# locuslab/mpc.pytorch

Measured on AMD Instinct MI355X. Metric: LQR problem-steps/sec (batch*T/s), n_state=12 n_ctrl=4 T=50, higher is better.
Workload: dtype f32

## Files before the change

include/mpc_lqr.h:

```cpp
#ifndef MPC_LQR_H
#define MPC_LQR_H

#include <stdint.h>

#ifdef __cplusplus
extern "C" {
#endif

#define MPC_LQR_ABI_VERSION 9

enum { MPC_F32 = 0, MPC_F64 = 1 };
enum { MPC_BOUND_NONE = 0, MPC_BOUND_SCALAR = 1, MPC_BOUND_TENSOR = 2 };
enum {
    MPC_OK = 0,
    MPC_E_DIMS = -1,
    MPC_E_NULL = -2,
    MPC_E_DTYPE = -3,
    MPC_E_LAUNCH = -4,
    MPC_E_ARG = -5,
    MPC_E_UNSUPPORTED = -6
};
enum {
    MPC_ST_PNQP_UNCONVERGED = 1,
    MPC_ST_NONFINITE = 2,
// ... 65 lines not shown
    void *k;
} mpc_lqr_outputs;

int mpc_lqr_abi_version(void);
const char *mpc_lqr_build_info(void);
const char *mpc_lqr_last_error(void);

int64_t mpc_lqr_workspace_bytes(const mpc_lqr_problem *p);

int mpc_lqr_step(const mpc_lqr_problem *p, const mpc_lqr_options *o, const mpc_lqr_outputs *out,
                 void *workspace, int64_t workspace_bytes, int impl, void *stream);

int mpc_lqr_step_route(const mpc_lqr_problem *p, const mpc_lqr_options *o, const mpc_lqr_outputs *out,
                       const void *workspace, int64_t workspace_bytes, int impl, int *ring);

int mpc_lqr_qp_record(const mpc_lqr_problem *p, const mpc_lqr_options *o, int impl, int64_t *offset_bytes, int64_t *st, int64_t *sb);

int mpc_lqr_impl_supported(const mpc_lqr_problem *p, const mpc_lqr_options *o, int impl);

int mpc_lqr_sweep(const mpc_lqr_problem *p, const mpc_lqr_options *o, const mpc_lqr_outputs *out,
                  void *stream);

int mpc_lqr_rollout(const mpc_lqr_problem *p, const mpc_lqr_options *o, const mpc_lqr_outputs *out,
                    const void *old_costs_in, void *stream);

int mpc_lqr_kkt_grads(const mpc_lqr_problem *p,
                      const void *dx, const void *du, const void *dl_dx, const void *dl_du,
                      void *dC, void *dc, void *dF, void *df, void *dx_init, void *stream);

enum { MPC_KKT_GRADS_DPP16 = 1, MPC_KKT_GRADS_WAVE = 2, MPC_KKT_GRADS_GENERIC = 3 };
// ... 106 lines not shown
```

mpc.pytorch_amd/csrc/capi.hip:

```cpp
#include <algorithm>
#include <cmath>
#include <cstdio>
#include <cstdlib>
#include <cstring>
#include <string>

#include "lqr_common.h"

namespace mpclqr {
static thread_local std::string g_last_error;
void set_last_error(const char *msg) { g_last_error = msg ? msg : ""; }

static int fail(int code, const char *msg)
{
    set_last_error(msg);
    return code;
}

struct DeviceFacts {
    int ring_force;
    int simds;
    int ring40_force;
    bool sticky;
};
static const DeviceFacts &device_facts()
{
    static DeviceFacts f = [] {
        DeviceFacts d;
        d.ring_force = 0;
        d.ring40_force = 0;
        d.simds = 1024;
        hipDeviceProp_t prop;
        int dev = 0;
        if (hipGetDevice(&dev) == hipSuccess && hipGetDeviceProperties(&prop, dev) == hipSuccess && prop.multiProcessorCount > 0)
            d.simds = prop.multiProcessorCount * 4;
        const char *force = getenv("MPC_DPP16_RING");
        if (force && (force[0] == '2' || force[0] == '4')) d.ring_force = force[0] - '0';
        const char *force40 = getenv("MPC_MFMA40_RING");
        if (force40 && (force40[0] == '2' || force40[0] == '3')) d.ring40_force = force40[0] - '0';
        d.sticky = getenv("MPC_DPP16_RING_DYNAMIC") == nullptr;
        return d;
    }();
    return f;
}
static int dpp16_ring_force()
{
    const DeviceFacts &f = device_facts();
    if (f.sticky) return f.ring_force;
    const char *force = getenv("MPC_DPP16_RING");
    return (force && (force[0] == '2' || force[0] == '4')) ? force[0] - '0' : 0;
}

static int mfma40_ring(const StepParams<float> &sp)
{
    const DeviceFacts &f = device_facts();
    int force = f.ring40_force;
    if (!f.sticky) {
        const char *e = getenv("MPC_MFMA40_RING");
        force = (e && (e[0] == '2' || e[0] == '3')) ? e[0] - '0' : 0;
    }
    if (force) return force;
    if (sp.bound_mode != MPC_BOUND_NONE) return sp.B > f.simds ? 2 : 3;
    return (sp.B > f.simds && sp.B <= f.simds + f.simds / 2) ? 2 : 3;
}

// ... 299 lines not shown
    sp.gate = sp.status;
    sp.Kk = nullptr;
    if (!sp.K || !sp.k) {
        const WsLayout w = ws_layout<real>(MPC_IMPL_GENERIC, sp.T, sp.B, sp.ns, sp.nc);
        sp.K = (real *)((char *)workspace + w.K);
        sp.k = (real *)((char *)workspace + w.k);
    }
    return launch_step_generic<real>(sp, sp.sweep_only ? 1 : 3, st);
}

static int launch_routed(const StepRoute &r, const StepParams<float> &q, hipStream_t st)
{
    switch (r.kernel) {
    case MPC_IMPL_GENERIC: return launch_step_generic<float>(q, r.phase, st);
    case MPC_IMPL_MFMA16: return launch_step_mfma16(q, st);
    case MPC_IMPL_DPP16: return r.ring == 2 ? launch_step_dpp16_ring2(q, st) : launch_step_dpp16(q, st);
    case MPC_IMPL_TINY: return launch_step_tiny<float>(q, st);
    case MPC_IMPL_MFMA40: return r.ring == 2 ? launch_step_mfma40_ring2(q, st) : launch_step_mfma40(q, st);
    case MPC_IMPL_WAVE1: return launch_step_wave1(q, st);
    case MPC_IMPL_MFMA40_PAD: return r.pad16 ? launch_step_mfma40_pad16(q, st) : launch_step_mfma40_pad4(q, st);
    case MPC_IMPL_DPP16_PAD: return launch_step_dpp16_pad(q, st);
    case MPC_IMPL_MFMA40_NARROW: return r.pad16 ? launch_step_mfma40_narrow16(q, st) : launch_step_mfma40_narrow4(q, st);
    }
    return MPC_E_ARG;
}
static int launch_routed(const StepRoute &r, const StepParams<double> &q, hipStream_t st)
{
    switch (r.kernel) {
    case MPC_IMPL_GENERIC: return launch_step_generic<double>(q, r.phase, st);
    case MPC_IMPL_MFMA16: return launch_step_mfma16(q, st);
    case MPC_IMPL_TINY: return launch_step_tiny<double>(q, st);
// ... 238 lines not shown
    if (!p) return 0;
    return status_scratch_offset(p) + (int64_t)p->B * 4 + 256;
}

int mpc_lqr_step(const mpc_lqr_problem *p, const mpc_lqr_options *o, const mpc_lqr_outputs *out,
                 void *workspace, int64_t workspace_bytes, int impl, void *stream)
{
    const int rc = check_step(p, o, out);
    if (rc) return rc;
    if (p->B == 0) return MPC_OK;
    hipStream_t st = (hipStream_t)stream;
    return p->dtype == MPC_F32 ? step_impl<float>(p, o, out, workspace, workspace_bytes, impl, 3, nullptr, st)
                               : step_impl<double>(p, o, out, workspace, workspace_bytes, impl, 3, nullptr, st);
}

int mpc_lqr_step_route(const mpc_lqr_problem *p, const mpc_lqr_options *o, const mpc_lqr_outputs *out, const void *workspace,
                       int64_t workspace_bytes, int impl, int *ring)
{
    const int rc = check_step(p, o, out);
    if (rc) return rc;
    if (ring) *ring = 0;
    if (p->B == 0) return 0;
    return p->dtype == MPC_F32 ? route_query<float>(p, o, out, workspace, workspace_bytes, impl, ring)
                               : route_query<double>(p, o, out, workspace, workspace_bytes, impl, ring);
}

int mpc_lqr_impl_supported(const mpc_lqr_problem *p, const mpc_lqr_options *o, int impl)
{
    if (!p || check_problem(p, false, false) != MPC_OK || check_options(p, o) != MPC_OK) return 0;
    if (impl < MPC_IMPL_GENERIC || impl > MPC_IMPL_MFMA40_NARROW) return 0;
// ... 453 lines not shown
```

mpc.pytorch_amd/csrc/lqr_common.h:

```cpp
#pragma once
#include <hip/hip_runtime.h>
#include <stdint.h>
#include "../../include/mpc_lqr.h"
#include "lqr_params.h"

namespace mpclqr {

void set_last_error(const char *msg);

enum { MPC_IMPL_AUTO = 0, MPC_IMPL_GENERIC = 1, MPC_IMPL_MFMA16 = 2, MPC_IMPL_DPP16 = 3, MPC_IMPL_TINY = 4, MPC_IMPL_MFMA40 = 5,
       MPC_IMPL_WAVE1 = 6, MPC_IMPL_MFMA40_PAD = 7, MPC_IMPL_DPP16_PAD = 8,
       MPC_IMPL_MFMA40_NARROW = 9 };

struct StepRoute {
    int code; const char *msg;
    int kernel;
    int phase;
    int ring;
    bool pad16;
    bool needs_resolve;
    int64_t K_off, k_off;
    int64_t Kk_off, status_off;
    int64_t qp_off, qp_st, qp_sb;
};
// ... 33 lines not shown
                                                real *bd, void *flags, void *host_flags, int host_tag, const int *status,
                                                hipStream_t st);
template <typename real> int launch_du_norm_reference(int T, int B, int nc, const real *u, const real *new_u, real *out, hipStream_t st);
template <typename real> int launch_env_linearize(const EnvDesc<real> &env, long N, const real *x, const real *u,
                                                  real *F, real *f, hipStream_t st);
int64_t env_param_grad_workspace_bytes(int64_t N);
template <typename real> int launch_env_param_grad(const EnvDesc<real> &env, long N, const real *x, const real *u,
                                                   const real *gF, const real *gf, real *gparams, double *ws, hipStream_t st);
size_t generic_lds_bytes(int ns, int nc, size_t elem);
template <typename real> int launch_slew_augment(const mpc_lqr_problem *p, double gamma, real *aC, real *ac, real *aF, real *af, hipStream_t st);

bool dpp16_supported(const StepParams<float> &p);
int launch_step_dpp16(const StepParams<float> &p, hipStream_t st);
int launch_step_dpp16_ring2(const StepParams<float> &p, hipStream_t st);
bool dpp16_pad_supported(const StepParams<float> &p);
int launch_step_dpp16_pad(const StepParams<float> &p, hipStream_t st);
bool kkt_dpp16_supported(const StepParams<float> &p, const float *dx, const float *du, const float *dl_dx,
                         const float *dC, const float *dF);
int launch_kkt_dpp16(const StepParams<float> &p, const float *dx, const float *du, const float *dl_dx, float *dC,
                     float *dc, float *dF, float *df, float *dx_init, hipStream_t st);

bool kkt_fused_dpp16_supported(const StepParams<float> &p, const float *dl_dx, const float *dl_du, const float *dC,
                               const float *dF, const float *ws);
int64_t kkt_fused_dpp16_workspace_bytes(int T, int B);
bool kkt_fused_dpp16_pad_supported(const StepParams<float> &p, const float *ws);
int launch_kkt_fused_dpp16_pad(const StepParams<float> &p, const float *dl_dx, const float *dl_du, float *dC, float *dc, float *dF,
                               float *df, float *dx_init, float *dx_out, float *du_out, float *ws, float decay, int max_ls,
                               hipStream_t st);
int launch_kkt_fused_dpp16(const StepParams<float> &p, const float *dl_dx, const float *dl_du, float *dC, float *dc, float *dF,
                           float *df, float *dx_init, float *dx_out, float *du_out, float *ws, float decay, int max_ls,
// ... 76 lines not shown
```

mpc.pytorch_amd/csrc/lqr_dpp16.hip:

```cpp
#include <string>
#include "lqr_common.h"

#define MPC_DEV __device__ __forceinline__
#define DPPM " row_mask:0xf bank_mask:0xf\n"

namespace mpclqr {
namespace wv {
typedef float f32x4 __attribute__((ext_vector_type(4)));
MPC_DEV int lane() { return (int)threadIdx.x; }
MPC_DEV int problem() { return (int)blockIdx.x; }
MPC_DEV unsigned long long clock() { return (unsigned long long)clock64(); }
MPC_DEV float rcp(float x) { return __builtin_amdgcn_rcpf(x); }
MPC_DEV void pin(float &x) { asm volatile("" : "+v"(x)); }
MPC_DEV bool uniform(bool c) { return c; }
MPC_DEV int uniform(int v) { return v; }
MPC_DEV bool any(bool c) { return __ballot(c) != 0ull; }
MPC_DEV unsigned long long ballot(bool c) { return __ballot(c); }
MPC_DEV float readlane(float x, int l) { return __int_as_float(__builtin_amdgcn_readlane(__float_as_int(x), __builtin_amdgcn_readfirstlane(l))); }
MPC_DEV double readlane_f64(double x, int l)
{
    const unsigned long long b = __double_as_longlong(x);
    const int ll = __builtin_amdgcn_readfirstlane(l);
    const unsigned lo = (unsigned)__builtin_amdgcn_readlane((int)(unsigned)b, ll), hi = (unsigned)__builtin_amdgcn_readlane((int)(unsigned)(b >> 32), ll);
    return __longlong_as_double(((unsigned long long)hi << 32) | lo);
// ... 272 lines not shown
}
MPC_DEV double row_sum_f64(double x)
{
    x += mov_dpp_f64<0xB1>(x);
    x += mov_dpp_f64<0x4E>(x);
    x += mov_dpp_f64<0x141>(x);
    x += mov_dpp_f64<0x140>(x);
    return x;
}

#ifndef MPC_DPP16_NSTAGE
#define MPC_DPP16_NSTAGE 4
#endif
#ifdef MPC_KF_LDS_BYTES
#define MPC_DPP16_LDS (MPC_KF_LDS_BYTES)
#else
#define MPC_DPP16_LDS (MPC_DPP16_NSTAGE * 9216)
#endif
#ifndef MPC_KKT16_NSTAGE
#define MPC_KKT16_NSTAGE 4
#endif
#if !defined(MPC_DPP16_WITH_KKT) && !defined(MPC_DPP16_NO_KKT) && MPC_DPP16_NSTAGE == 4
#define MPC_DPP16_WITH_KKT 1
#endif
__shared__ __attribute__((aligned(16))) char g_stage16[MPC_DPP16_LDS];
typedef __attribute__((address_space(3))) void lds_void_t;
typedef __attribute__((address_space(1))) const void glb_void_t;
#ifndef MPC_DPP16_C_AUX
#define MPC_DPP16_C_AUX 2
#endif
// ... 243 lines not shown
    return true;
}

#endif

#ifndef MPC_DPP16_PAD_KKT
#ifdef MPC_DPP16_PAD
#define MPC_DPP16_LAUNCH launch_step_dpp16_pad
bool dpp16_pad_supported(const StepParams<float> &p)
{
    return p.ns >= 1 && p.ns <= 12 && p.nc >= 1 && p.nc <= 4 && p.T >= 1 && p.max_ls >= 1 && p.max_ls <= 16 && !p.env.kind;
}
#define MPC_DPP16_TAKES(p) dpp16_pad_supported(p)
#elif MPC_DPP16_NSTAGE == 4
#define MPC_DPP16_LAUNCH launch_step_dpp16
#else
#define MPC_DPP16_LAUNCH launch_step_dpp16_ring2
bool dpp16_supported(const StepParams<float> &p);
#endif
int MPC_DPP16_LAUNCH(const StepParams<float> &p, hipStream_t st)
{
#ifndef MPC_DPP16_TAKES
#define MPC_DPP16_TAKES(p) dpp16_supported(p)
#endif
    if (!MPC_DPP16_TAKES(p)) { set_last_error(dpp16::PADK ? "dpp16 (padded): needs fp32, n_state <= 12, n_ctrl <= 4, max_linesearch_iter <= 16" : "dpp16: needs n_state = 12, n_ctrl = 4, fp32, 16-byte aligned blocks"); return MPC_E_DIMS; }
    if (!p.Kk || (uintptr_t)p.Kk % 16 != 0) { set_last_error("dpp16: gain workspace missing or misaligned"); return MPC_E_NULL; }
    if (!p.sweep_only && (!p.new_x || !p.new_u)) { set_last_error("dpp16: new_x / new_u is NULL"); return MPC_E_NULL; }
    static_assert(MPC_DPP16_LDS == dpp16::LDS_TOTAL, "LDS layout out of sync");
    const dim3 grid((p.B + 3) / 4), block(64);
    if (p.bound_mode != MPC_BOUND_NONE) hipLaunchKernelGGL((lqr_step_dpp16_kernel<2>), grid, block, 0, st, p);
    else if (p.zero_mask) hipLaunchKernelGGL((lqr_step_dpp16_kernel<1>), grid, block, 0, st, p);
    else if (p.T <= dpp16::RG_STEPS) hipLaunchKernelGGL((lqr_step_dpp16_kernel<0>), grid, block, 0, st, p);
    else hipLaunchKernelGGL((lqr_step_dpp16_kernel<3>), grid, block, 0, st, p);
    hipError_t e = hipGetLastError();
    if (e != hipSuccess) {
        set_last_error((std::string("lqr_step_dpp16_kernel: ") + hipGetErrorString(e)).c_str());
        return MPC_E_LAUNCH;
    }
    return MPC_OK;
}
#endif

}
```

mpc.pytorch_amd/csrc/lqr_dpp16_body.h:

```cpp
#pragma once
#include <math.h>
#include "lqr_params.h"
#include "lqr_small_math.h"

#ifndef MPC_STAT
#define MPC_STAT(i)
#endif

#ifndef MPC_DEVM
#define MPC_DEVM MPC_DEV
#endif

#ifndef MPC_DPP16_NSTAGE
#define MPC_DPP16_NSTAGE 4
#endif
#ifndef MPC_DPP16_QP_WARM
#define MPC_DPP16_QP_WARM 0
#endif

#ifdef MPC_DPP16_PAD
#define MPC_DPP16_PADK 1
#else
#define MPC_DPP16_PADK 0
#endif
// ... 194 lines not shown
    fr_out[2] = wv::bcast<8>(mv) != 0.f; fr_out[3] = wv::bcast<12>(mv) != 0.f;
    converged = conv != 0.f;
    return (int)it_ret;
}

enum {
    SC = 0, SF = 4096, SR = 7168, SG = 8192, STAGE_BYTES = 9216, NSTAGE = MPC_DPP16_NSTAGE, AHEAD = NSTAGE - 1,
    R_c = 0, R_tau = 64, R_f = 128, R_qs = 176, R_lo = 192, R_hi = 208,
    LDS_TOTAL = NSTAGE * STAGE_BYTES,
#if defined(MPC_PAD_PROBE_DUP) && MPC_DPP16_PADK
    DMA_SWEEP = 48
#else
    DMA_SWEEP = MPC_DPP16_PADK ? 32 : 8
#endif
};
#if defined(MPC_PAD_PROBE_DUP) && MPC_DPP16_PADK
#define MPC_PAD_NF 12
#define MPC_PAD_NC 32
#else
#define MPC_PAD_NF 12
#define MPC_PAD_NC 16
#endif
template <int MODE, bool DIRECT> struct RollDma { enum { N = (MPC_DPP16_PADK ? MPC_PAD_NF + 4 : 3 + 1) + (rgm(MODE) ? 0 : 1) + (DIRECT ? (MPC_DPP16_PADK ? MPC_PAD_NC : 4) : (con(MODE) ? 1 : 0)) }; };
template <int MODE, bool DIRECT> struct RollRing {
    enum {
        BYTES = DIRECT ? (int)STAGE_BYTES : (con(MODE) ? 6144 : (rgm(MODE) ? 4096 : 5120)),
#ifdef MPC_DPP16_RSLOTS
        SLOTS = DIRECT ? (int)NSTAGE : (MPC_DPP16_RSLOTS),
#else
        SLOTS = DIRECT ? (int)NSTAGE : (int)LDS_TOTAL / (con(MODE) ? 6144 : (rgm(MODE) ? 4096 : 5120)),
// ... 15 lines not shown
    wv::lds_sync();
    for (unsigned off = 16u * (unsigned)lane; off + 16 <= bytes; off += 1024) wv::lds_store_f32x4(off, f32x4{0.f, 0.f, 0.f, 0.f});
    wv::lds_sync();
}

MPC_DEV int quarter_swizzle(int row) { return (row >> 1) & 3; }
MPC_DEV int src_granule_rows(int g) { return (g & ~3) | ((g & 3) ^ quarter_swizzle(g >> 2)); }
MPC_DEV int src_granule_cols(int g, int problem_slot) { return g ^ ((problem_slot & 1) << 2); }
MPC_DEV int src_granule_C(int g, int problem_slot)
{
#ifdef MPC_DPP16_NO_CPERM
    problem_slot = 0;
#endif
    const int R = (g >> 2) ^ (problem_slot & 3);
    return 4 * R + ((g & 3) ^ quarter_swizzle(R));
}

struct Lane {
    int lane, p, j;
    int pb;
    int b0;
    bool live;
    bool isu;
    bool ovalid;
    float padd[4];
    int a;
    int aCq[4];
    int aCcol;
    int aFe, aFo;
    int aFq[4];
// ... 205 lines not shown
        else if (K == 1) { MPC_PAD_C(8); MPC_PAD_C(9); MPC_PAD_C(10); MPC_PAD_C(11); MPC_PAD_C(12); MPC_PAD_C(13); MPC_PAD_C(14); MPC_PAD_C(15); }
        else if (K == 2) { MPC_PAD_F(0); MPC_PAD_F(1); MPC_PAD_F(2); MPC_PAD_F(3); MPC_PAD_F(4); MPC_PAD_F(5); MPC_PAD_F(6); MPC_PAD_F(7); }
        else { MPC_PAD_F(8); MPC_PAD_F(9); MPC_PAD_F(10); MPC_PAD_F(11); MPC_PAD_R(0); MPC_PAD_R(1); MPC_PAD_R(2); MPC_PAD_R(3); }
    } else {
        if (K == 0) { MPC_PAD_F(0); MPC_PAD_F(1); MPC_PAD_F(2); MPC_PAD_F(3); MPC_PAD_F(4); MPC_PAD_F(5); }
        else if (K == 1) { MPC_PAD_F(6); MPC_PAD_F(7); MPC_PAD_F(8); MPC_PAD_F(9); MPC_PAD_F(10); MPC_PAD_F(11); }
        else if (K == 2) { MPC_PAD_R(0); MPC_PAD_R(1); MPC_PAD_R(2); MPC_PAD_R(3); }
    }
#undef MPC_PAD_C
#undef MPC_PAD_F
#undef MPC_PAD_R
}
#endif

template <int MODE, bool ROLL, bool DIRECT>
MPC_DEV void stage_issue(const Dma &d, unsigned mid)
{
#ifdef MPC_DPP16_PAD
    pad_part<MODE, ROLL, DIRECT, 0>(d, mid); pad_part<MODE, ROLL, DIRECT, 1>(d, mid);
    pad_part<MODE, ROLL, DIRECT, 2>(d, mid); pad_part<MODE, ROLL, DIRECT, 3>(d, mid);
    if (ROLL && !rgm(MODE)) {
        if (DIRECT) wv::dma16_at<0>(d.g_ptr - 1024, mid + (SG - SF));
        else wv::dma16_at<-1024>(d.g_ptr, mid);
    }
    if (ROLL && !DIRECT && con(MODE)) wv::dma16_at<-2048>(d.g2_ptr, mid);
    return;
#endif
    if (!ROLL || DIRECT) {
        wv::dma16_at<-4096, wv::DMA_C>(d.c_ptr[0], mid);
        wv::dma16_at<-3072, wv::DMA_C>(d.c_ptr[1], mid);
        wv::dma16_at<-2048, wv::DMA_C>(d.c_ptr[2], mid);
        wv::dma16_at<-1024, wv::DMA_C>(d.c_ptr[3], mid);
    }
    wv::dma16_at<0, ROLL ? wv::DMA_LAST : wv::DMA_PLAIN>(d.f_ptr[0], mid);
    wv::dma16_at<1024, ROLL ? wv::DMA_LAST : wv::DMA_PLAIN>(d.f_ptr[1], mid);
    wv::dma16_at<2048, ROLL ? wv::DMA_LAST : wv::DMA_PLAIN>(d.f_ptr[2], mid);
    wv::dma16_at<3072>(d.r_ptr, mid);
    if (ROLL && !rgm(MODE)) {
        if (DIRECT) {
            wv::dma16_at<0>(d.g_ptr - 1024, mid + (SG - SF));
        } else {
            wv::dma16_at<-1024>(d.g_ptr, mid);
            if (con(MODE)) wv::dma16_at<-2048>(d.g2_ptr, mid);
        }
    }
}

template <int MODE, bool ROLL, bool DIRECT>
MPC_DEV void stage_move(Dma &d, bool move_f)
{
#ifdef MPC_DPP16_PAD
// ... 27 lines not shown
        if (con(MODE) && !DIRECT) d.g2_ptr += d.g2_step;
    }
}

template <int K, int ND> MPC_DEV void tail_wait(int rem)
{
    if (K == 0 || rem >= K) wv::dma_wait<K * ND>();
    else tail_wait<(K > 0 ? K - 1 : 0), ND>(rem);
}

template <int MODE, bool ROLL, bool DIRECT> struct Feed {
    Dma &d;
    unsigned mid;
    bool on;
    bool move_f;
    template <int K> MPC_DEVM void part()
    {
        if (!on) return;
#ifdef MPC_DPP16_PAD
        pad_part<MODE, ROLL, DIRECT, K>(d, mid);
        if (ROLL && !DIRECT) {
            if (K == 2) {
                if (!rgm(MODE)) wv::dma16_at<-1024>(d.g_ptr, mid);
                if (con(MODE)) wv::dma16_at<-2048>(d.g2_ptr, mid);
            } else if (K == 3) {
                stage_move<MODE, ROLL, DIRECT>(d, move_f);
            }
        } else if (K == 3) {
            if (ROLL && !rgm(MODE)) wv::dma16_at<0>(d.g_ptr - 1024, mid + (SG - SF));
            stage_move<MODE, ROLL, DIRECT>(d, move_f);
        }
        return;
#endif
        enum { NC = (!ROLL || DIRECT) ? 4 : 0 };
        if (ROLL && !DIRECT) {
            if (K == 0) {
                wv::dma16_at<0, wv::DMA_LAST>(d.f_ptr[0], mid);
                wv::dma16_at<1024, wv::DMA_LAST>(d.f_ptr[1], mid);
            } else if (K == 1) {
                wv::dma16_at<2048, wv::DMA_LAST>(d.f_ptr[2], mid);
                wv::dma16_at<3072>(d.r_ptr, mid);
            } else if (K == 2) {
                if (!rgm(MODE)) wv::dma16_at<-1024>(d.g_ptr, mid);
                if (con(MODE)) wv::dma16_at<-2048>(d.g2_ptr, mid);
            } else {
                stage_move<MODE, ROLL, DIRECT>(d, move_f);
            }
        } else {
            if (K == 0) {
                wv::dma16_at<-4096, wv::DMA_C>(d.c_ptr[0], mid);
                wv::dma16_at<-3072, wv::DMA_C>(d.c_ptr[1], mid);
            } else if (K == 1) {
                wv::dma16_at<-2048, wv::DMA_C>(d.c_ptr[2], mid);
                wv::dma16_at<-1024, wv::DMA_C>(d.c_ptr[3], mid);
            } else if (K == 2) {
// ... 380 lines not shown
    const f32x4 r = s.rec;
    const float k0 = wv::bcast<12>(r[0]), k1 = wv::bcast<12>(r[1]), k2 = wv::bcast<12>(r[2]), k3 = wv::bcast<12>(r[3]);
    const int a = L.a;
    s.kk = a == 0 ? k0 : (a == 1 ? k1 : (a == 2 ? k2 : k3));
    const float q00 = wv::bcast<13>(r[2]);
    const float q01 = wv::bcast<13>(r[0]), q11 = wv::bcast<13>(r[1]);
    const float q02 = wv::bcast<14>(r[0]), q12 = wv::bcast<14>(r[1]), q22 = wv::bcast<14>(r[2]);
    const float q03 = wv::bcast<15>(r[0]), q13 = wv::bcast<15>(r[1]), q23 = wv::bcast<15>(r[2]), q33 = wv::bcast<15>(r[3]);
    s.Sr[0] = a == 0 ? q00 : (a == 1 ? q01 : (a == 2 ? q02 : q03));
    s.Sr[1] = a == 0 ? q01 : (a == 1 ? q11 : (a == 2 ? q12 : q13));
    s.Sr[2] = a == 0 ? q02 : (a == 1 ? q12 : (a == 2 ? q22 : q23));
    s.Sr[3] = a == 0 ? q03 : (a == 1 ? q13 : (a == 2 ? q23 : q33));
}

template <int MODE, bool DIRECT>
MPC_DEV void ro_read(RoStage &s, const P &p, const Lane &L, int t, int slot, unsigned zm)
{
    const unsigned base = stage_mid<MODE, true, DIRECT>(slot) - SF;
    const unsigned mrec = base + RollRing<MODE, DIRECT>::MADJ;
    const unsigned gain = base + RollRing<MODE, DIRECT>::GADJ;
    s.cj = 0.f;
    if (DIRECT) {
#pragma unroll
        for (int q = 0; q < 4; ++q) {
            const f32x4 v = wv::lds_f32x4(base + L.aCq[q]);
            s.Cr[4 * q] = v[0]; s.Cr[4 * q + 1] = v[1]; s.Cr[4 * q + 2] = v[2]; s.Cr[4 * q + 3] = v[3];
        }
        s.cj = wv::lds_f32(base + L.aRec + R_c);
    } else {
#pragma unroll
        for (int b = 0; b < 4; ++b) s.Sr[b] = rgm(MODE) ? 0.f : wv::lds_f32(gain + L.aS[b]);
        if (con(MODE)) {
            const f32x4 mc = wv::lds_f32x4(L.j == 12 ? mrec + L.aMcol : gain + L.aGcol);
            const unsigned fm = wv::f32_bits(wv::lds_f32(gain + L.aFm));
#pragma unroll
            for (int a = 0; a < 4; ++a) s.Mc[a] = (L.j == 12 || !((fm >> a) & 1u)) ? mc[a] : 0.f;
        }
    }
#pragma unroll
    for (int q = 0; q < 4; ++q) {
        const f32x4 v = wv::lds_f32x4(base + L.aFq[q]);
        s.Fr[4 * q] = v[0]; s.Fr[4 * q + 1] = v[1]; s.Fr[4 * q + 2] = v[2]; s.Fr[4 * q + 3] = v[3];
    }
    s.fj = p.f ? wv::lds_f32(base + L.aRecF) : 0.f;
    if (!rgm(MODE)) {
#pragma unroll
        for (int jj = 0; jj < 12; ++jj) s.Kr[jj] = wv::lds_f32(gain + L.aKrow + 16 * jj);
        if (con(MODE)) {
            const unsigned fm = wv::f32_bits(wv::lds_f32(gain + L.aFm));
            const bool free_a = ((fm >> L.a) & 1u) != 0u;
#pragma unroll
            for (int jj = 0; jj < 12; ++jj) s.Kr[jj] = free_a ? s.Kr[jj] : 0.f;
        }
        s.kk = wv::lds_f32(gain + L.aKrow + 192);
    } else {
        s.kk = 0.f;
// ... 9 lines not shown
            s.lo = pad ? 0.f : p.lo_s;
            s.hi = pad ? 0.f : p.hi_s;
        }
    }
    s.zm = ((zm >> (8 * L.a)) & 0xffu) != 0u;
}

struct RoState {
    float xs;
    float cost, du2;
    float alpha;
    float pred;
    float viol;
    float *out;
    bool price_on;
    float xs1, cost1, du21;
    float *out1;
};

template <int MODE>
MPC_DEV float control_law(const P &p, const Lane &L, const RoStage &s, float xs, float alpha, float &e, float &dx)
{
    dx = L.isu ? 0.f : xs - s.tb;
    float un;
    if (rgm(MODE)) {
        const float mult = L.j == 12 ? alpha : dx;
        un = s.tb + wv::quad_sums(s.rec[0] * mult, s.rec[1] * mult, s.rec[2] * mult, s.rec[3] * mult, L.j);
    } else {
        un = fmaf(alpha, s.kk, s.tb);
        wv::dot_bcast12(un, dx, s.Kr);
// ... 134 lines not shown
        st.cost = 0.f;
        st.du2 = 0.f;
        st.pred = 0.f;
        st.out = L.out0;
        if (PAIR) {
            st.xs1 = x0;
            st.cost1 = 0.f;
            st.du21 = 0.f;
            st.out1 = L.scr0;
        }
    }
    st.price_on = MULTI || wv::any(st.alpha != 1.f);
    const bool use_zm = con(MODE) && p.zero_mask != nullptr;
    enum { NS = RollRing<MODE, DIRECT>::SLOTS, LA = NS - 1, ND = RollDma<MODE, DIRECT>::N };
    static_assert((LA - 1) * ND + 2 * LA < 64, "vmcnt is 6 bits");
    unsigned zq[NS];
#pragma unroll
    for (int i = 0; i < NS; ++i) zq[i] = 0u;
    dma_seek<MODE, true, DIRECT>(d, p, L, wave);
    pad_clear(L.lane);
#pragma unroll
    for (int i = 0; i < LA; ++i) {
        if (i < T) {
            stage_issue<MODE, true, DIRECT>(d, stage_mid<MODE, true, DIRECT>(i));
            stage_move<MODE, true, DIRECT>(d, i + 1 <= T - 2);
            if (use_zm) zq[i] = zm_pick(L, zm_fetch(p, L, i));
        }
    }
    for (int t0 = 0; t0 < T; t0 += NS) {
#pragma unroll
        for (int i = 0; i < NS; ++i) {
            const int t = t0 + i;
            if (t < T) {
                PROF_MARK(7);
                if (T - 1 - t >= LA - 1) wv::dma_wait<(LA - 1) * ND>();
                else tail_wait<(LA >= 2 ? LA - 2 : 0), ND>(T - 1 - t);
                PROF_MARK(4);
                RoStage s;
                ro_read<MODE, DIRECT>(s, p, L, t, i, zq[i]);
                if (rgm(MODE)) {
                    s.rec = gain_get(G, t);
                    if (!DIRECT && st.price_on) rg_price_terms(s, L);
                }
                PROF_MARK(5);
                const int tn = t + LA;
                ZmRaw zr = {{0u, 0u, 0u, 0u}};
                if (use_zm && tn < T) zr = zm_fetch(p, L, tn);
                Feed<MODE, true, DIRECT> feed = {d, stage_mid<MODE, true, DIRECT>((i + LA) % NS), tn < T, tn + 1 <= T - 2};
                PROF_MARK(6);
                if (MULTI) {
                    feed.template part<0>(); feed.template part<1>(); feed.template part<2>(); feed.template part<3>();
                    trials_step<MODE, DIRECT>(p, L, s, tr, nt, t);
                } else {
                    rollout_step<MODE, DIRECT, CHECK, PAIR>(p, L, s, st, t, feed);
                }
                if (use_zm) zq[(i + LA) % NS] = zm_pick(L, zr);
            }
        }
    }
    wv::dma_wait<0>();
    if (MULTI) {
#pragma unroll
        for (int k = 0; k < MAX_TRIALS; ++k)
// ... 196 lines not shown
    ss.vv = 0.f;
    ss.oc = 0.0;
    ss.w0 = 0.0;
    ss.warm = 0;
    ss.qp_total = 0;
    ss.status = 0;
    ss.asym = 0.f;
    ss.cmax = 0.f;
    ss.kprev[0] = ss.kprev[1] = ss.kprev[2] = ss.kprev[3] = 0.f;
    ss.rec_step = (long)p.B * 64;
    ss.rec = p.Kk + ((long)(T - 1) * p.B + L.pb) * 64 + 4 * L.j;
    ss.rec2_step = (long)p.B * 4;
    ss.rec2 = p.Kk + (long)T * p.B * 64 + ((long)(T - 1) * p.B + L.pb) * 4;
    {
        unsigned zq[NSTAGE] = {};
        dma_seek<MODE, false, false>(d, p, L, wave);
        pad_clear(L.lane);
#pragma unroll
        for (int i = 0; i < AHEAD; ++i) {
            const int ti = T - 1 - i;
            if (ti >= 0) {
                stage_issue<MODE, false, false>(d, stage_mid<MODE, false, false>(i));
                stage_move<MODE, false, false>(d, ti <= T - 2);
                if (MODE == 1) zq[i] = zm_pick(L, zm_fetch(p, L, ti));
            }
        }
        for (int k0 = 0; k0 < T; k0 += NSTAGE) {
#pragma unroll
            for (int i = 0; i < NSTAGE; ++i) {
                const int t = T - 1 - (k0 + i);
                if (t >= 0) {
                    PROF_MARK(3);
                    if (t >= AHEAD - 1) wv::dma_wait<(AHEAD - 1) * DMA_SWEEP>();
                    else wv::dma_wait<0>();
                    PROF_MARK(0);
                    SwStage s;
                    sw_read<MODE>(s, p, L, t, i, zq[i], ss.asym, ss.cmax);
                    PROF_MARK(1);
                    ZmRaw zr = {{0u, 0u, 0u, 0u}};
                    if (MODE == 1 && t >= AHEAD) zr = zm_fetch(p, L, t - AHEAD);
                    Feed<MODE, false, false> feed = {d, stage_mid<MODE, false, false>((i + AHEAD) % NSTAGE), t >= AHEAD, true};
                    PROF_MARK(2);
                    sweep_step<MODE>(p, L, s, ss, t, feed, G PROF_PASS);
                    if (MODE == 1) zq[(i + AHEAD) % NSTAGE] = zm_pick(L, zr);
                }
            }
        }
        wv::dma_wait<0>();
    }
    PROF_MARK_ALL(8);
    const double old_cost_d = wv::row_sum_f64(ss.oc);
    const float old_cost = (float)old_cost_d;
    if (!p.c_symmetric) ss.status |= MPC_ST_C_TESTED | (wv::row_max(ss.asym) > 1e-5f * wv::row_max(ss.cmax) ? (int)MPC_ST_C_ASYMMETRIC : 0);

    if (p.sweep_only) {
        if (L.j == 0) {
            if (p.old_costs) p.old_costs[L.pb] = old_cost;
            if (p.qp_iters) p.qp_iters[L.pb] = ss.qp_total;
            if (p.status) p.status[L.pb] = ss.status;
        }
        return;
    }
    wv::fence_own_stores();

    RoState rs;
    rs.viol = 0.f;
    float full2 = 0.f;
    if (p.on_dynamics) {
        line_search<MODE, false, false>(p, L, d, wave, G, rs, old_cost, old_cost_d + ss.w0, full2 PROF_PASS);
    } else {
        line_search<MODE, false, true>(p, L, d, wave, G, rs, old_cost, old_cost_d + ss.w0, full2 PROF_PASS);
        bool off = wv::row_sum(rs.viol > 0.f ? 1.f : 0.f) > 0.f;
        {
            const long o0 = L.isu ? 0 : (long)(L.out0 - p.new_x);
            const float xi = p.x_init[o0], n0 = p.cur_x[o0];
            float r = fabsf(xi - n0) - 1e-5f * (1.f + fabsf(n0));
            r = (r == r) ? r : 1.f;
            const bool mine = !L.isu && (!PADK || L.ovalid) && r > 0.f;
            const bool off0 = wv::row_sum(mine ? 1.f : 0.f) > 0.f;
            if (wv::any(off0)) {
                const f32x4 zero4 = {0.f, 0.f, 0.f, 0.f};
// ... 343 lines not shown
                    s1.cx = wv::lds_f32(base + SR + L.p * 256 + 128 + 4 * jx);
#pragma unroll
                    for (int a = 0; a < 4; ++a) { s1.lo[a] = 0.f; s1.hi[a] = 0.f; }
                    if (MASKED) {
                        if (p.bound_mode == MPC_BOUND_TENSOR) {
                            const f32x4 l = wv::lds_f32x4(base + SR + L.p * 256 + R_lo);
                            const f32x4 h = wv::lds_f32x4(base + SR + L.p * 256 + R_hi);
#pragma unroll
                            for (int a = 0; a < 4; ++a) { s1.lo[a] = l[a]; s1.hi[a] = h[a]; }
                        } else {
#pragma unroll
                            for (int a = 0; a < 4; ++a) { s1.lo[a] = p.lo_s; s1.hi[a] = p.hi_s; }
                        }
                    }
                }
                Feed<0, false, false> feed = {d, stage_mid<0, false, false>((i + AHEAD) % NSTAGE), t >= AHEAD, true};
                feed.template part<0>();

                float ln = s1.cx;
                wv::dot_bcast16(ln, s1.tj, s1.Cc);
                if (!last) wv::dot_bcast12(ln, lam, s1.Fc);

                float Q[16];
                float q = -s1.rj;
#pragma unroll
                for (int r = 0; r < 16; ++r) Q[r] = s1.Cc[r];
                if (!last) {
                    float Y[12] = {0.f, 0.f, 0.f, 0.f, 0.f, 0.f, 0.f, 0.f, 0.f, 0.f, 0.f, 0.f};
                    wv::sched_fence();
#pragma unroll
                    for (int m = 0; m < 12; ++m) outer_acc(Y, Vc[m], s1.Fc[m]);
// ... 369 lines not shown
```

mpc.pytorch_amd/mpc/_native.py:

```python
import ctypes
import math
import os

import torch

_HERE = os.path.dirname(os.path.abspath(__file__))
LIB_NAME = "libmpc_lqr_hip.so"

MPC_F32, MPC_F64 = 0, 1
BOUND_NONE, BOUND_SCALAR, BOUND_TENSOR = 0, 1, 2
ST_PNQP_UNCONVERGED, ST_NONFINITE, ST_NOMINAL_OFF_DYNAMICS, ST_C_ASYMMETRIC, ST_QUU_SINGULAR, ST_C_TESTED = 1, 2, 4, 8, 16, 32
IMPL_AUTO, IMPL_GENERIC, IMPL_MFMA16, IMPL_DPP16, IMPL_TINY, IMPL_MFMA40, IMPL_WAVE1, IMPL_MFMA40_PAD, IMPL_DPP16_PAD = 0, 1, 2, 3, 4, 5, 6, 7, 8
IMPL_MFMA40_NARROW = 9

KKT_NONE, KKT_DPP16, KKT_DPP16_PAD, KKT_MFMA40, KKT_MFMA40_PAD16, KKT_MFMA40_PAD4 = 0, 1, 2, 3, 4, 5
KKT_MFMA40_NARROW16, KKT_MFMA40_NARROW4 = 6, 7
KKT_PREFER_NARROW = 100
KKT_GRADS_DPP16, KKT_GRADS_WAVE, KKT_GRADS_GENERIC = 1, 2, 3

ABI_VERSION = 9

_vp, _i32, _i64, _f64 = ctypes.c_void_p, ctypes.c_int32, ctypes.c_int64, ctypes.c_double


# ... 143 lines not shown
                for Wb in zip(self.weights, self.biases) for t in Wb]
        e = self._complete([(W.data_ptr(), b.data_ptr()) for W, b in zip(keep[0::2], keep[1::2])])
        nbytes = int(load().mpc_mlp_workspace_bytes(ctypes.byref(e)))
        ws = torch.empty(nbytes, device=like.device, dtype=torch.uint8)
        keep.append(ws)
        return e, ws, nbytes, keep


class Outputs(ctypes.Structure):
    _fields_ = [("new_x", _vp), ("new_u", _vp), ("costs", _vp), ("old_costs", _vp), ("full_du_norm", _vp),
                ("alpha_du_norm", _vp), ("alphas", _vp), ("qp_iters", _vp), ("status", _vp),
                ("K", _vp), ("k", _vp)]


EXPORTS = ("mpc_lqr_abi_version", "mpc_lqr_build_info", "mpc_lqr_last_error", "mpc_lqr_workspace_bytes",
           "mpc_lqr_step", "mpc_lqr_step_route", "mpc_lqr_impl_supported", "mpc_lqr_qp_record", "mpc_lqr_sweep", "mpc_lqr_rollout", "mpc_lqr_kkt_grads", "mpc_lqr_kkt_prepare",
           "mpc_pnqp", "mpc_pnqp_lu", "mpc_traj_cost", "mpc_env_traj_cost", "mpc_env_linearize", "mpc_select_best",
           "mpc_env_param_grad_workspace_bytes", "mpc_env_param_grad",
           "mpc_mlp_workspace_bytes", "mpc_mlp_rollout", "mpc_mlp_linearize", "mpc_mlp_linearize_carry",
           "mpc_mlp_param_grad_workspace_bytes", "mpc_mlp_param_grad",
           "mpc_mlp_supported", "mpc_lqr_kkt_fused_supported", "mpc_lqr_kkt_fused_workspace_bytes", "mpc_lqr_kkt_fused",
           "mpc_du_norm_reference", "mpc_slew_augment",
           "mpc_lqr_kkt_shared_supported", "mpc_lqr_kkt_shared_workspace_bytes", "mpc_lqr_kkt_grads_shared",
           "mpc_lqr_kkt_fused_route", "mpc_lqr_kkt_grads_route",
           "mpc_lqr_kkt_fused_kernel", "mpc_lqr_kkt_fused_kernel_route", "mpc_lqr_kkt_fused_kernel_workspace_bytes")

_lib = None


class NativeLibraryMissing(RuntimeError):
    pass
# ... 10 lines not shown
    path = lib_path()
    if not os.path.exists(path):
        raise NativeLibraryMissing(
            "%s not found at %s -- build it with `python __graft_entry__.py` "
            "(hipcc --offload-arch=gfx950); there is no CPU fallback." % (LIB_NAME, path))
    L = ctypes.CDLL(path)
    for name in EXPORTS:
        getattr(L, name)
    L.mpc_lqr_build_info.restype = ctypes.c_char_p
    L.mpc_lqr_last_error.restype = ctypes.c_char_p
    L.mpc_lqr_workspace_bytes.restype = _i64
    L.mpc_lqr_workspace_bytes.argtypes = [ctypes.POINTER(Problem)]
    PP, OP, UP = ctypes.POINTER(Problem), ctypes.POINTER(Options), ctypes.POINTER(Outputs)
    L.mpc_lqr_step.argtypes = [PP, OP, UP, _vp, _i64, ctypes.c_int, _vp]
    L.mpc_lqr_step_route.argtypes = [PP, OP, UP, _vp, _i64, ctypes.c_int, ctypes.POINTER(ctypes.c_int)]
    L.mpc_lqr_impl_supported.argtypes = [PP, OP, ctypes.c_int]
    L.mpc_lqr_qp_record.argtypes = [PP, OP, ctypes.c_int] + [ctypes.POINTER(_i64)] * 3
    L.mpc_lqr_sweep.argtypes = [PP, OP, UP, _vp]
    L.mpc_lqr_rollout.argtypes = [PP, OP, UP, _vp, _vp]
    L.mpc_du_norm_reference.argtypes = [ctypes.c_int] * 4 + [_vp] * 4
    L.mpc_lqr_kkt_grads.argtypes = [PP] + [_vp] * 10
    L.mpc_lqr_kkt_prepare.argtypes = [ctypes.c_int] * 5 + [_vp, _vp, _vp, OP, _vp, _vp, _vp]
    L.mpc_lqr_kkt_fused_supported.argtypes = [PP, OP]
    L.mpc_lqr_kkt_fused_workspace_bytes.restype = _i64
    L.mpc_lqr_kkt_fused_workspace_bytes.argtypes = [PP]
    L.mpc_lqr_kkt_fused.argtypes = [PP, OP] + [_vp] * 11 + [_i64, _vp]
    L.mpc_lqr_kkt_fused_route.argtypes = [PP, OP] + [_vp] * 11 + [_i64]
    L.mpc_lqr_kkt_grads_route.argtypes = [PP] + [_vp] * 9
    L.mpc_lqr_kkt_fused_kernel.argtypes = [PP, OP, ctypes.c_int] + [_vp] * 11 + [_i64, _vp]
    L.mpc_lqr_kkt_fused_kernel_route.argtypes = [PP, OP, ctypes.c_int] + [_vp] * 11 + [_i64]
# ... 866 lines not shown
```

Before: 2.255 billion.

## Keep selected F blocks resident in LDS between sweep and rollout in dpp16

Adds a resident-F variant of the dpp16 ring2 kernel. During the backward sweep it copies up to seven dynamics-matrix (F) stage blocks per wavefront into extra LDS, and the forward rollout/line search reads those blocks from LDS instead of re-fetching F from global memory, with the slots staggered across waves. The intent is to cut global memory traffic in the rollout phase. The cost is more LDS per wave (up to 40 KiB), which may limit occupancy, plus a new compile variant, a routing heuristic enabled by default when the batch nearly fills the SIMDs, and a launch counter.

After: 2.291 billion (median of 6 runs). 1.6% higher.

```diff
diff --git a/include/mpc_lqr.h b/include/mpc_lqr.h
--- a/include/mpc_lqr.h
+++ b/include/mpc_lqr.h
@@ -103,6 +103,8 @@
 int mpc_lqr_step_route(const mpc_lqr_problem *p, const mpc_lqr_options *o, const mpc_lqr_outputs *out,
                        const void *workspace, int64_t workspace_bytes, int impl, int *ring);
 
+int64_t mpc_lqr_resident_launches(void);
+
 int mpc_lqr_qp_record(const mpc_lqr_problem *p, const mpc_lqr_options *o, int impl, int64_t *offset_bytes, int64_t *st, int64_t *sb);
 
 int mpc_lqr_impl_supported(const mpc_lqr_problem *p, const mpc_lqr_options *o, int impl);
diff --git a/mpc.pytorch_amd/csrc/capi.hip b/mpc.pytorch_amd/csrc/capi.hip
--- a/mpc.pytorch_amd/csrc/capi.hip
+++ b/mpc.pytorch_amd/csrc/capi.hip
@@ -1,4 +1,5 @@
 #include <algorithm>
+#include <atomic>
 #include <cmath>
 #include <cstdio>
 #include <cstdlib>
@@ -22,6 +23,7 @@
     int simds;
     int ring40_force;
     bool sticky;
+    int resident;
 };
 static const DeviceFacts &device_facts()
 {
@@ -39,6 +41,8 @@
         const char *force40 = getenv("MPC_MFMA40_RING");
         if (force40 && (force40[0] == '2' || force40[0] == '3')) d.ring40_force = force40[0] - '0';
         d.sticky = getenv("MPC_DPP16_RING_DYNAMIC") == nullptr;
+        const char *res = getenv("MPC_DPP16_RESIDENT");
+        d.resident = (res && (res[0] == '0' || res[0] == '1')) ? res[0] - '0' : -1;
         return d;
     }();
     return f;
@@ -49,6 +53,24 @@
     if (f.sticky) return f.ring_force;
     const char *force = getenv("MPC_DPP16_RING");
     return (force && (force[0] == '2' || force[0] == '4')) ? force[0] - '0' : 0;
+}
+
+#ifndef MPC_DPP16_RESIDENT_DEFAULT
+#define MPC_DPP16_RESIDENT_DEFAULT 1
+#endif
+static std::atomic<int64_t> g_resident_launches{0};
+static bool dpp16_resident(const StepParams<float> &q)
+{
+    const DeviceFacts &f = device_facts();
+    int on = f.resident;
+    if (!f.sticky) {
+        const char *e = getenv("MPC_DPP16_RESIDENT");
+        on = (e && (e[0] == '0' || e[0] == '1')) ? e[0] - '0' : -1;
+    }
+    const int waves = (q.B + 3) / 4;
+    if (on < 0) on = (MPC_DPP16_RESIDENT_DEFAULT && 16 * (long)waves > 15 * (long)f.simds) ? 1 : 0;
+    return on != 0 && q.bound_mode == MPC_BOUND_NONE && !q.zero_mask && q.T >= 2 && q.T <= 64  && !q.sweep_only &&
+           (q.B + 3) / 4 <= f.simds;
 }
 
 static int mfma40_ring(const StepParams<float> &sp)
@@ -378,7 +400,13 @@
     switch (r.kernel) {
     case MPC_IMPL_GENERIC: return launch_step_generic<float>(q, r.phase, st);
     case MPC_IMPL_MFMA16: return launch_step_mfma16(q, st);
-    case MPC_IMPL_DPP16: return r.ring == 2 ? launch_step_dpp16_ring2(q, st) : launch_step_dpp16(q, st);
+    case MPC_IMPL_DPP16:
+        if (r.ring == 2 && dpp16_resident(q)) {
+            g_resident_launches.fetch_add(1, std::memory_order_relaxed);
+            return launch_step_dpp16_res(q, st);
+        }
+        if (r.ring == 2) return launch_step_dpp16_ring2(q, st);
+        return launch_step_dpp16(q, st);
     case MPC_IMPL_TINY: return launch_step_tiny<float>(q, st);
     case MPC_IMPL_MFMA40: return r.ring == 2 ? launch_step_mfma40_ring2(q, st) : launch_step_mfma40(q, st);
     case MPC_IMPL_WAVE1: return launch_step_wave1(q, st);
@@ -647,6 +675,8 @@
                                : step_impl<double>(p, o, out, workspace, workspace_bytes, impl, 3, nullptr, st);
 }
 
+int64_t mpc_lqr_resident_launches(void) { return g_resident_launches.load(std::memory_order_relaxed); }
+
 int mpc_lqr_step_route(const mpc_lqr_problem *p, const mpc_lqr_options *o, const mpc_lqr_outputs *out, const void *workspace,
                        int64_t workspace_bytes, int impl, int *ring)
 {
diff --git a/mpc.pytorch_amd/csrc/lqr_common.h b/mpc.pytorch_amd/csrc/lqr_common.h
--- a/mpc.pytorch_amd/csrc/lqr_common.h
+++ b/mpc.pytorch_amd/csrc/lqr_common.h
@@ -71,6 +71,7 @@
 int launch_step_dpp16(const StepParams<float> &p, hipStream_t st);
 int launch_step_dpp16_ring2(const StepParams<float> &p, hipStream_t st);
 bool dpp16_pad_supported(const StepParams<float> &p);
+int launch_step_dpp16_res(const StepParams<float> &p, hipStream_t st);
 int launch_step_dpp16_pad(const StepParams<float> &p, hipStream_t st);
 bool kkt_dpp16_supported(const StepParams<float> &p, const float *dx, const float *du, const float *dl_dx,
                          const float *dC, const float *dF);
diff --git a/mpc.pytorch_amd/csrc/lqr_dpp16.hip b/mpc.pytorch_amd/csrc/lqr_dpp16.hip
--- a/mpc.pytorch_amd/csrc/lqr_dpp16.hip
+++ b/mpc.pytorch_amd/csrc/lqr_dpp16.hip
@@ -310,6 +310,9 @@
 #endif
 #ifdef MPC_KF_LDS_BYTES
 #define MPC_DPP16_LDS (MPC_KF_LDS_BYTES)
+#elif defined(MPC_DPP16_RESIDENT)
+#define MPC_DPP16_LDS (MPC_DPP16_NSTAGE * 9216 + 7 * 3072)
+static_assert(MPC_DPP16_LDS <= 40960, "resident F: a wavefront's quarter of the CU's 160 KiB");
 #else
 #define MPC_DPP16_LDS (MPC_DPP16_NSTAGE * 9216)
 #endif
@@ -583,6 +586,9 @@
 #define MPC_DPP16_TAKES(p) dpp16_pad_supported(p)
 #elif MPC_DPP16_NSTAGE == 4
 #define MPC_DPP16_LAUNCH launch_step_dpp16
+#elif defined(MPC_DPP16_RESIDENT)
+#define MPC_DPP16_LAUNCH launch_step_dpp16_res
+bool dpp16_supported(const StepParams<float> &p);
 #else
 #define MPC_DPP16_LAUNCH launch_step_dpp16_ring2
 bool dpp16_supported(const StepParams<float> &p);
@@ -595,12 +601,17 @@
     if (!MPC_DPP16_TAKES(p)) { set_last_error(dpp16::PADK ? "dpp16 (padded): needs fp32, n_state <= 12, n_ctrl <= 4, max_linesearch_iter <= 16" : "dpp16: needs n_state = 12, n_ctrl = 4, fp32, 16-byte aligned blocks"); return MPC_E_DIMS; }
     if (!p.Kk || (uintptr_t)p.Kk % 16 != 0) { set_last_error("dpp16: gain workspace missing or misaligned"); return MPC_E_NULL; }
     if (!p.sweep_only && (!p.new_x || !p.new_u)) { set_last_error("dpp16: new_x / new_u is NULL"); return MPC_E_NULL; }
-    static_assert(MPC_DPP16_LDS == dpp16::LDS_TOTAL, "LDS layout out of sync");
+    static_assert(MPC_DPP16_LDS == dpp16::LDS_RES_TOTAL, "LDS layout out of sync");
     const dim3 grid((p.B + 3) / 4), block(64);
+#ifdef MPC_DPP16_RESIDENT
+    if (p.bound_mode != MPC_BOUND_NONE || p.zero_mask || p.T > dpp16::RG_STEPS) { set_last_error("dpp16 (resident F): mode 0 only"); return MPC_E_ARG; }
+    hipLaunchKernelGGL((lqr_step_dpp16_kernel<0>), grid, block, 0, st, p);
+#else
     if (p.bound_mode != MPC_BOUND_NONE) hipLaunchKernelGGL((lqr_step_dpp16_kernel<2>), grid, block, 0, st, p);
     else if (p.zero_mask) hipLaunchKernelGGL((lqr_step_dpp16_kernel<1>), grid, block, 0, st, p);
     else if (p.T <= dpp16::RG_STEPS) hipLaunchKernelGGL((lqr_step_dpp16_kernel<0>), grid, block, 0, st, p);
     else hipLaunchKernelGGL((lqr_step_dpp16_kernel<3>), grid, block, 0, st, p);
+#endif
     hipError_t e = hipGetLastError();
     if (e != hipSuccess) {
         set_last_error((std::string("lqr_step_dpp16_kernel: ") + hipGetErrorString(e)).c_str());
diff --git a/mpc.pytorch_amd/csrc/lqr_dpp16_body.h b/mpc.pytorch_amd/csrc/lqr_dpp16_body.h
--- a/mpc.pytorch_amd/csrc/lqr_dpp16_body.h
+++ b/mpc.pytorch_amd/csrc/lqr_dpp16_body.h
@@ -232,6 +232,40 @@
     DMA_SWEEP = MPC_DPP16_PADK ? 32 : 8
 #endif
 };
+#ifdef MPC_DPP16_RESIDENT
+#define MPC_DPP16_RESK 1
+#else
+#define MPC_DPP16_RESK 0
+#endif
+#ifndef MPC_DPP16_RES_T0
+#define MPC_DPP16_RES_T0 0
+#endif
+#ifndef MPC_DPP16_RES_STRIDE
+#define MPC_DPP16_RES_STRIDE 7
+#endif
+constexpr bool RESK = MPC_DPP16_RESK != 0;
+enum { RES_STAGES = 7, RES_BLOCK = 3072, RES_T0 = MPC_DPP16_RES_T0, RES_STRIDE = MPC_DPP16_RES_STRIDE,
+       RES_BASE = LDS_TOTAL, LDS_RES_TOTAL = LDS_TOTAL + (RESK ? RES_STAGES * RES_BLOCK : 0) };
+static_assert(!RESK || (!PADK && LDS_RES_TOTAL <= 40960 && RES_STRIDE >= 1), "resident F: a quarter of a CU's LDS, exact 12/4 only");
+MPC_DEV unsigned long long res_mask(int wave, int T)
+{
+    const int nF = T - 1;
+    if (nF <= RES_STAGES) return nF > 0 ? (1ull << nF) - 1ull : 0ull;
+    const int t0 = RES_T0 >= 0 ? (int)RES_T0 : (nF + RES_T0 > 0 ? nF + RES_T0 : 0);
+    unsigned long long m = 0ull;
+#pragma unroll
+    for (int k = 0; k < RES_STAGES; ++k) {
+        const int t = t0 + wave % RES_STRIDE + k * RES_STRIDE;
+        if (t < nF) m |= 1ull << t;
+    }
+    return m;
+}
+MPC_DEV int res_slot(unsigned long long mask, int t)
+{
+    return ((mask >> t) & 1ull) ? (int)__builtin_popcountll(mask & ((1ull << t) - 1ull)) : -1;
+}
+MPC_DEV bool res_alias(unsigned long long mask, int t, int T) { return t >= T - 1 || ((mask >> t) & 1ull) != 0ull; }
+
 #if defined(MPC_PAD_PROBE_DUP) && MPC_DPP16_PADK
 #define MPC_PAD_NF 12
 #define MPC_PAD_NC 32
@@ -277,6 +311,24 @@
 #endif
     const int R = (g >> 2) ^ (problem_slot & 3);
     return 4 * R + ((g & 3) ^ quarter_swizzle(R));
+}
+struct ResLane { int src[3], dst; };
+MPC_DEV void res_lane_init(ResLane &R, int lane)
+{
+#pragma unroll
+    for (int k = 0; k < 3; ++k) {
+        const int G = 64 * k + lane, slot = G / 48, gi = G - 48 * slot;
+        R.src[k] = SF + 16 * (48 * slot + (src_granule_rows(gi) ^ ((slot & 1) << 2)));
+    }
+    R.dst = RES_BASE + 16 * lane;
+}
+MPC_DEV void res_keep(const ResLane &R, int slot, int k)
+{
+    const unsigned sb = (unsigned)(slot * (int)STAGE_BYTES), db = (unsigned)(k * (int)RES_BLOCK + R.dst);
+    const f32x4 v0 = wv::lds_f32x4(sb + (unsigned)R.src[0]), v1 = wv::lds_f32x4(sb + (unsigned)R.src[1]), v2 = wv::lds_f32x4(sb + (unsigned)R.src[2]);
+    wv::lds_store_f32x4(db, v0);
+    wv::lds_store_f32x4(db + 1024, v1);
+    wv::lds_store_f32x4(db + 2048, v2);
 }
 
 struct Lane {
@@ -512,7 +564,7 @@
 #endif
 
 template <int MODE, bool ROLL, bool DIRECT>
-MPC_DEV void stage_issue(const Dma &d, unsigned mid)
+MPC_DEV void stage_issue(const Dma &d, unsigned mid, bool alias_f = false)
 {
 #ifdef MPC_DPP16_PAD
     pad_part<MODE, ROLL, DIRECT, 0>(d, mid); pad_part<MODE, ROLL, DIRECT, 1>(d, mid);
@@ -530,9 +582,15 @@
         wv::dma16_at<-2048, wv::DMA_C>(d.c_ptr[2], mid);
         wv::dma16_at<-1024, wv::DMA_C>(d.c_ptr[3], mid);
     }
-    wv::dma16_at<0, ROLL ? wv::DMA_LAST : wv::DMA_PLAIN>(d.f_ptr[0], mid);
-    wv::dma16_at<1024, ROLL ? wv::DMA_LAST : wv::DMA_PLAIN>(d.f_ptr[1], mid);
-    wv::dma16_at<2048, ROLL ? wv::DMA_LAST : wv::DMA_PLAIN>(d.f_ptr[2], mid);
+    if (RESK && ROLL && !DIRECT && MODE == 0 && alias_f) {
+        wv::dma16_at<0>(d.r_ptr + 3072, mid);
+        wv::dma16_at<1024>(d.r_ptr + 2048, mid);
+        wv::dma16_at<2048>(d.r_ptr + 1024, mid);
+    } else {
+        wv::dma16_at<0, ROLL ? wv::DMA_LAST : wv::DMA_PLAIN>(d.f_ptr[0], mid);
+        wv::dma16_at<1024, ROLL ? wv::DMA_LAST : wv::DMA_PLAIN>(d.f_ptr[1], mid);
+        wv::dma16_at<2048, ROLL ? wv::DMA_LAST : wv::DMA_PLAIN>(d.f_ptr[2], mid);
+    }
     wv::dma16_at<3072>(d.r_ptr, mid);
     if (ROLL && !rgm(MODE)) {
         if (DIRECT) {
@@ -590,6 +648,7 @@
     unsigned mid;
     bool on;
     bool move_f;
+    bool alias_f;
     template <int K> MPC_DEVM void part()
     {
         if (!on) return;
@@ -610,11 +669,18 @@
 #endif
         enum { NC = (!ROLL || DIRECT) ? 4 : 0 };
         if (ROLL && !DIRECT) {
+            const bool alias = RESK && MODE == 0 && alias_f;
             if (K == 0) {
-                wv::dma16_at<0, wv::DMA_LAST>(d.f_ptr[0], mid);
-                wv::dma16_at<1024, wv::DMA_LAST>(d.f_ptr[1], mid);
+                if (alias) {
+                    wv::dma16_at<0>(d.r_ptr + 3072, mid);
+                    wv::dma16_at<1024>(d.r_ptr + 2048, mid);
+                } else {
+                    wv::dma16_at<0, wv::DMA_LAST>(d.f_ptr[0], mid);
+                    wv::dma16_at<1024, wv::DMA_LAST>(d.f_ptr[1], mid);
+                }
             } else if (K == 1) {
-                wv::dma16_at<2048, wv::DMA_LAST>(d.f_ptr[2], mid);
+                if (alias) wv::dma16_at<2048>(d.r_ptr + 1024, mid);
+                else wv::dma16_at<2048, wv::DMA_LAST>(d.f_ptr[2], mid);
                 wv::dma16_at<3072>(d.r_ptr, mid);
             } else if (K == 2) {
                 if (!rgm(MODE)) wv::dma16_at<-1024>(d.g_ptr, mid);
@@ -1025,9 +1091,10 @@
 }
 
 template <int MODE, bool DIRECT>
-MPC_DEV void ro_read(RoStage &s, const P &p, const Lane &L, int t, int slot, unsigned zm)
+MPC_DEV void ro_read(RoStage &s, const P &p, const Lane &L, int t, int slot, unsigned zm, int res_k = -1)
 {
     const unsigned base = stage_mid<MODE, true, DIRECT>(slot) - SF;
+    const unsigned fbase = (RESK && MODE == 0 && !DIRECT && res_k >= 0) ? (unsigned)((int)RES_BASE + res_k * (int)RES_BLOCK - (int)SF) : base;
     const unsigned mrec = base + RollRing<MODE, DIRECT>::MADJ;
     const unsigned gain = base + RollRing<MODE, DIRECT>::GADJ;
     s.cj = 0.f;
@@ -1050,7 +1117,7 @@
     }
 #pragma unroll
     for (int q = 0; q < 4; ++q) {
-        const f32x4 v = wv::lds_f32x4(base + L.aFq[q]);
+        const f32x4 v = wv::lds_f32x4(fbase + L.aFq[q]);
         s.Fr[4 * q] = v[0]; s.Fr[4 * q + 1] = v[1]; s.Fr[4 * q + 2] = v[2]; s.Fr[4 * q + 3] = v[3];
     }
     s.fj = p.f ? wv::lds_f32(base + L.aRecF) : 0.f;
@@ -1090,6 +1157,7 @@
     float viol;
     float *out;
     bool price_on;
+    unsigned long long resmask;
     float xs1, cost1, du21;
     float *out1;
 };
@@ -1254,6 +1322,7 @@
     const bool use_zm = con(MODE) && p.zero_mask != nullptr;
     enum { NS = RollRing<MODE, DIRECT>::SLOTS, LA = NS - 1, ND = RollDma<MODE, DIRECT>::N };
     static_assert((LA - 1) * ND + 2 * LA < 64, "vmcnt is 6 bits");
+    constexpr bool RES = RESK && MODE == 0 && !DIRECT;
     unsigned zq[NS];
 #pragma unroll
     for (int i = 0; i < NS; ++i) zq[i] = 0u;
@@ -1262,7 +1331,7 @@
 #pragma unroll
     for (int i = 0; i < LA; ++i) {
         if (i < T) {
-            stage_issue<MODE, true, DIRECT>(d, stage_mid<MODE, true, DIRECT>(i));
+            stage_issue<MODE, true, DIRECT>(d, stage_mid<MODE, true, DIRECT>(i), RES && res_alias(st.resmask, i, T));
             stage_move<MODE, true, DIRECT>(d, i + 1 <= T - 2);
             if (use_zm) zq[i] = zm_pick(L, zm_fetch(p, L, i));
         }
@@ -1277,7 +1346,7 @@
                 else tail_wait<(LA >= 2 ? LA - 2 : 0), ND>(T - 1 - t);
                 PROF_MARK(4);
                 RoStage s;
-                ro_read<MODE, DIRECT>(s, p, L, t, i, zq[i]);
+                ro_read<MODE, DIRECT>(s, p, L, t, i, zq[i], RES ? res_slot(st.resmask, t) : -1);
                 if (rgm(MODE)) {
                     s.rec = gain_get(G, t);
                     if (!DIRECT && st.price_on) rg_price_terms(s, L);
@@ -1286,7 +1355,7 @@
                 const int tn = t + LA;
                 ZmRaw zr = {{0u, 0u, 0u, 0u}};
                 if (use_zm && tn < T) zr = zm_fetch(p, L, tn);
-                Feed<MODE, true, DIRECT> feed = {d, stage_mid<MODE, true, DIRECT>((i + LA) % NS), tn < T, tn + 1 <= T - 2};
+                Feed<MODE, true, DIRECT> feed = {d, stage_mid<MODE, true, DIRECT>((i + LA) % NS), tn < T, tn + 1 <= T - 2, RES && tn < T && res_alias(st.resmask, tn, T)};
                 PROF_MARK(6);
                 if (MULTI) {
                     feed.template part<0>(); feed.template part<1>(); feed.template part<2>(); feed.template part<3>();
@@ -1513,6 +1582,9 @@
     ss.rec2 = p.Kk + (long)T * p.B * 64 + ((long)(T - 1) * p.B + L.pb) * 4;
     {
         unsigned zq[NSTAGE] = {};
+        ResLane rl;
+        if (RESK && MODE == 0) res_lane_init(rl, lane);
+        const unsigned long long resmask = (RESK && MODE == 0) ? res_mask(wave, T) : 0ull;
         dma_seek<MODE, false, false>(d, p, L, wave);
         pad_clear(L.lane);
 #pragma unroll
@@ -1535,10 +1607,14 @@
                     PROF_MARK(0);
                     SwStage s;
                     sw_read<MODE>(s, p, L, t, i, zq[i], ss.asym, ss.cmax);
+                    if (RESK && MODE == 0) {
+                        const int rk = res_slot(resmask, t);
+                        if (rk >= 0) res_keep(rl, i, rk);
+                    }
                     PROF_MARK(1);
                     ZmRaw zr = {{0u, 0u, 0u, 0u}};
                     if (MODE == 1 && t >= AHEAD) zr = zm_fetch(p, L, t - AHEAD);
-                    Feed<MODE, false, false> feed = {d, stage_mid<MODE, false, false>((i + AHEAD) % NSTAGE), t >= AHEAD, true};
+                    Feed<MODE, false, false> feed = {d, stage_mid<MODE, false, false>((i + AHEAD) % NSTAGE), t >= AHEAD, true, false};
                     PROF_MARK(2);
                     sweep_step<MODE>(p, L, s, ss, t, feed, G PROF_PASS);
                     if (MODE == 1) zq[(i + AHEAD) % NSTAGE] = zm_pick(L, zr);
@@ -1564,6 +1640,7 @@
 
     RoState rs;
     rs.viol = 0.f;
+    rs.resmask = (RESK && MODE == 0) ? res_mask(wave, T) : 0ull;
     float full2 = 0.f;
     if (p.on_dynamics) {
         line_search<MODE, false, false>(p, L, d, wave, G, rs, old_cost, old_cost_d + ss.w0, full2 PROF_PASS);
@@ -1937,7 +2014,7 @@
                         }
                     }
                 }
-                Feed<0, false, false> feed = {d, stage_mid<0, false, false>((i + AHEAD) % NSTAGE), t >= AHEAD, true};
+                Feed<0, false, false> feed = {d, stage_mid<0, false, false>((i + AHEAD) % NSTAGE), t >= AHEAD, true, false};
                 feed.template part<0>();
 
                 float ln = s1.cx;
diff --git a/mpc.pytorch_amd/mpc/_native.py b/mpc.pytorch_amd/mpc/_native.py
--- a/mpc.pytorch_amd/mpc/_native.py
+++ b/mpc.pytorch_amd/mpc/_native.py
@@ -181,7 +181,7 @@
 
 
 EXPORTS = ("mpc_lqr_abi_version", "mpc_lqr_build_info", "mpc_lqr_last_error", "mpc_lqr_workspace_bytes",
-           "mpc_lqr_step", "mpc_lqr_step_route", "mpc_lqr_impl_supported", "mpc_lqr_qp_record", "mpc_lqr_sweep", "mpc_lqr_rollout", "mpc_lqr_kkt_grads", "mpc_lqr_kkt_prepare",
+           "mpc_lqr_step", "mpc_lqr_step_route", "mpc_lqr_resident_launches", "mpc_lqr_impl_supported", "mpc_lqr_qp_record", "mpc_lqr_sweep", "mpc_lqr_rollout", "mpc_lqr_kkt_grads", "mpc_lqr_kkt_prepare",
            "mpc_pnqp", "mpc_pnqp_lu", "mpc_traj_cost", "mpc_env_traj_cost", "mpc_env_linearize", "mpc_select_best",
            "mpc_env_param_grad_workspace_bytes", "mpc_env_param_grad",
            "mpc_mlp_workspace_bytes", "mpc_mlp_rollout", "mpc_mlp_linearize", "mpc_mlp_linearize_carry",
@@ -222,6 +222,8 @@
     PP, OP, UP = ctypes.POINTER(Problem), ctypes.POINTER(Options), ctypes.POINTER(Outputs)
     L.mpc_lqr_step.argtypes = [PP, OP, UP, _vp, _i64, ctypes.c_int, _vp]
     L.mpc_lqr_step_route.argtypes = [PP, OP, UP, _vp, _i64, ctypes.c_int, ctypes.POINTER(ctypes.c_int)]
+    L.mpc_lqr_resident_launches.restype = _i64
+    L.mpc_lqr_resident_launches.argtypes = []
     L.mpc_lqr_impl_supported.argtypes = [PP, OP, ctypes.c_int]
     L.mpc_lqr_qp_record.argtypes = [PP, OP, ctypes.c_int] + [ctypes.POINTER(_i64)] * 3
     L.mpc_lqr_sweep.argtypes = [PP, OP, UP, _vp]
```
